# PereUbu7/Variational-Self-Organizing-Maps

Hardware: AMD Instinct MI355X
Metric: training samples/sec per epoch (BMU+update), 128x128 map, 784-dim (higher is better)
Workload: dtype f32

## Files before the change

variational-self-organizing-maps_amd/csrc/vsom_device.hpp:

```cpp
#pragma once
#include "vsom_internal.hpp"

struct DistArgs {
    const float *xa;
    const float *xb;
    int ldx;
    const float *ma;
    const float *mb;
    int ldm;
    int L;
};

template <bool CLR>
__device__ __forceinline__ float vsom_resid(float x, float y, float m, float b)
{
    if (CLR) {
        float t = m * x;
        t = t + b;
        t = t - y;
        return t;
    }
    return m - x;
}

// ... 115 lines not shown
__device__ __forceinline__ void vsom_local_walk_with(DistFn dist, u64 width, u64 height, u64 start, int lane,
                                                     u64 &minIndexOut, float &minDistOut)
{
    const int g = lane >> 3, k = lane & 7;
    const u64 m1 = ~0ull;
    const u64 fsx = (g == 0 || g >= 6) ? m1 : ((g == 1 || g == 5) ? 0ull : 1ull);
    const u64 fsy = (g <= 2) ? 1ull : ((g == 3 || g == 7) ? 0ull : m1);

    u64 lastBMU = start;
    float minDist = dist(lastBMU, k);
    minDist = __shfl(minDist, 0);
    u64 minIndex = lastBMU;
    u64 lastMeasured = lastBMU;

    for (;;) {
        const u64 lmX = lastMeasured % width, lmY = lastMeasured / width;
        const u64 lbX = lastBMU % width, lbY = lastBMU / width;
        if (lastMeasured == lastBMU) {
            u64 cx = lmX + fsx;
            cx = cx < width - 1 ? cx : width - 1;
            u64 cy = lmY + fsy;
            cy = cy < height - 1 ? cy : height - 1;
            u64 node = cy * width + cx;
            float d = dist(node, k);
#pragma unroll
            for (int i = 0; i < 8; ++i) {
                float di = __shfl(d, i * 8);
                u64 ni = __shfl(node, i * 8);
                if (di < minDist) {
                    minDist = di;
                    minIndex = ni;
                }
            }
            if (minIndex == lastBMU)
                break;
            lastMeasured = minIndex;
        } else {
            if (lmX - lbX) {
                u64 cx = lmX + lmX - lbX;
                cx = cx < width - 1 ? cx : width - 1;
                u64 off = (u64)(long long)((g < 3 ? g : 0) - 1);
                u64 cy = lmY + off;
                cy = cy < height - 1 ? cy : height - 1;
                u64 node = cy * width + cx;
                float d = dist(node, k);
#pragma unroll
                for (int i = 0; i < 3; ++i) {
                    float di = __shfl(d, i * 8);
                    u64 ni = __shfl(node, i * 8);
                    if (di < minDist) {
                        minDist = di;
                        minIndex = ni;
                    }
                }
            }
            (void)lbY;
            if (minIndex == lastMeasured)
                break;
            lastBMU = lastMeasured;
            lastMeasured = minIndex;
        }
    }
    minIndexOut = minIndex;
    minDistOut = minDist;
}

template <bool CLR>
__device__ __forceinline__ void vsom_local_walk(const DistArgs &a, const float *xa, const float *xb, u64 width,
                                                u64 height, u64 start, int lane, u64 &minIndexOut, float &minDistOut)
{
    vsom_local_walk_with(
        [&](u64 node, int k) {
            return vsom_group_dist<CLR>(xa, xb, a.ma + (size_t)node * a.ldm, a.mb + (size_t)node * a.ldm, a.L, k);
        },
        width, height, start, lane, minIndexOut, minDistOut);
}

__device__ __forceinline__ void vsom_somindex(u64 idx, u64 W, u64 H, int &x, int &y)
{
    u64 xm = idx % W;
    x = (int)xm;
    y = (int)((idx - xm) / H);
}
```

variational-self-organizing-maps_amd/csrc/vsom_internal.hpp:

```cpp
#pragma once

#include <hip/hip_runtime.h>
#include <stdint.h>
#include <stddef.h>
#include <algorithm>
#include <map>
#include <string>
#include <tuple>
#include <vector>

#include "../../include/vsom_hip.h"
#include "vsom_buf.hpp"

typedef unsigned long long u64;

#define VSOM_CHAIN_MAX_WAVES 448

#define VSOM_TK 32

constexpr size_t VSOM_ROW_PAD = 32;
constexpr size_t VSOM_ONL_STATE_BYTES = 4352;

struct vsom_custom_state;

// ... 34 lines not shown
    DevBuf<int> cc_idx_alt, cc_inv_alt;
    DevBuf<unsigned> cc_meta_alt;
    hipEvent_t ev_rows_free = nullptr, ev_ahead = nullptr;
    bool rows_free_valid = false;
    bool ahead_valid = false;
    bool ahead_rows = false;
    size_t ahead_B = 0;
    bool ahead_cc = false, ahead_xi = false;
    const float *next_dev = nullptr;
    size_t next_dev_B = 0;
    bool next_dev_pending = false;
    PinnedBuf<float> mse;
    PinnedBuf<unsigned char> sch_host; DevBuf<unsigned char> sch_dev;
    PinnedBuf<float> sch_mse;
    DevBuf<int> pair_i, pair_j;

    DevBuf<u64> partial;
    DevBuf<unsigned char> nan0;

    DevBuf<u64> dd_hash; DevBuf<int> dd_rep, dd_list;
    bool dedupe = true;
    double dd_min_work = 2.0e10;
    bool tiny_lds_attr[12] = {};

    DevBuf<float> sl_G, sl_nrm; DevBuf<unsigned> sl_scal;
    DevBuf<float> sl_a2;
    DevBuf<int> sl_list;
    DevBuf<float> sl_tmin;
    PinnedBuf<unsigned> sl_fb;
    DevBuf<float> sl_fs, sl_fm;
    DevBuf<signed char> sl_xi; DevBuf<float> sl_l1;
    DevBuf<signed char> sl_q; DevBuf<double> sl_qscale, sl_qcorr;
    DevBuf<int4> sl_qfast;
    uint32_t sl_kp8 = 0;
    bool xi_valid = false;
    int sl_par = 0;
    int sl_skip = 0;
    unsigned sl_seq_seen = 0;
    int sl_fail_streak = 0;

    DevBuf<float2> cw;
    DevBuf<float> lut; PinnedBuf<float> lut_host;
    hipEvent_t lut_ev[2] = {nullptr, nullptr}; bool lut_ev_valid[2] = {false, false}; int lut_slot = 0;
    double lut_sigma = -1.0; uint32_t lut_w = 0, lut_h = 0;
    DevBuf<double> lutd; double lutd_sigma = -1.0;
    PinnedBuf<double> lutd_host; double lutd_host_sigma[2] = {-1.0, -1.0};
    hipEvent_t lutd_ev[2] = {nullptr, nullptr}; bool lutd_ev_valid[2] = {false, false}; int lutd_slot = 0;

    void *upd_module = nullptr, *upd_clr8 = nullptr;
    void *upd_quad[VSOM_QF_COUNT][VSOM_QV_COUNT] = {};
    bool mean_nt4 = false;
    int update_mode = VSOM_UPDATE_STRICT;
    bool use_chain = true;
    bool use_tiny = true;

    DevBuf<unsigned> cc_flags;
    DevBuf<int> cc_idx;
    DevBuf<int> cc_inv;
    DevBuf<unsigned> cc_meta;
    PinnedBuf<unsigned> cc_fb;
    unsigned cc_seen = 0;
    int cc_skip = 0;
    long cc_min_rows = 1024;
    bool cc_valid = false;
    uint32_t cpitch = 0;
    DevBuf<float> Xc;
    DevBuf<float> Mc;
    DevBuf<float> Uc_map, Uc_S;
    DevBuf<float4> Xq;
    DevBuf<unsigned> zq;
    bool xq_valid = false;
    uint32_t xq_bpad = 0, xq_quads = 0;

    struct PendingSigma {
        bool on = false;
        size_t B = 0;
        uint32_t bpad = 0;
        bool compact = false;
        VsomQuadVariant variant = VSOM_QV_STD;
        double sigma = 0.0;
    } sg;
    DevBuf<int> sg_inv; DevBuf<unsigned> sg_meta;
    DevBuf<u64> sg_bmu;
    int sigma_mode = VSOM_SIGMA_AUTO;
    unsigned sigma_unread = 0;
    bool sigma_shared = false;
    uint64_t sg_stats[3] = {0, 0, 0};

    DevBuf<float> v_dev;
    PinnedBuf<float> v_pinned;
    DevBuf<float> res_dev;
    DevBuf<u64> onl_state;
    DevBuf<float> onl_f;
    DevBuf<unsigned char> onl_img; DevBuf<float4> onl_nsc; DevBuf<float> onl_lb; DevBuf<unsigned> onl_u;
    DevBuf<float4> onl_xsc;
    DevBuf<unsigned char> onl_dirty;

    PinnedBuf<float> st_pinned;
    PinnedBuf<u64> out_pinned;
    DevBuf<unsigned char> q_scratch;
    PinnedBuf<unsigned char> q_pinned;
    DevBuf<double> umatrix;
    bool um_valid = false;

    uint32_t timing = 0;
    struct Ev { hipEvent_t a, b; int which; };
    std::vector<Ev> ev_live;
    std::vector<Ev> ev_pool;
    float t_ms[VSOM_T_COUNT] = {0};
    uint32_t t_cnt[VSOM_T_COUNT] = {0};

    bool in_group = false;

    vsom_custom_state *cu = nullptr;
};

void vsom_set_error(const std::string &msg);
int vsom_fail(int code, const std::string &msg);
#define VSOM_HIP_CHECK_AS(expr, what)                                                    \
    do {                                                                                 \
        hipError_t _e = (expr);                                                          \
        if (_e != hipSuccess) {                                                          \
            (void)hipGetLastError();                                                     \
            return vsom_fail(_e == hipErrorOutOfMemory ? VSOM_ERR_NOMEM : VSOM_ERR_HIP,  \
                             std::string(what) + ": " + hipGetErrorString(_e));          \
        }                                                                                \
    } while (0)
#define VSOM_HIP_CHECK(expr) VSOM_HIP_CHECK_AS(expr, #expr)
#define VSOM_ALLOC_CHECK(expr) VSOM_HIP_CHECK_AS(expr, "hipMalloc in " #expr)

struct TimerScope {
    vsom_ctx *c; int which; vsom_ctx::Ev ev; bool on;
    TimerScope(vsom_ctx *ctx, int w);
    ~TimerScope();
};

struct DistArgs;
DistArgs vsom_dist_args(const vsom_ctx *c);
struct VsomNodeGroups {
    size_t G, ng;
};
inline VsomNodeGroups vsom_node_groups(size_t ntiles, size_t rtiles, size_t maxg)
{
    const size_t want = std::min<size_t>({maxg, ntiles, std::max<size_t>(1, (2048 + rtiles - 1) / rtiles)});
    const size_t G = (ntiles + want - 1) / want;
    return {G, (ntiles + G - 1) / G};
}
int launch_stage_chunk(vsom_ctx *c, const float *x_dev, size_t B);
int ensure_chunk_capacity(vsom_ctx *c, size_t B);
bool vsom_can_stage_ahead(const vsom_ctx *c, size_t B);
int launch_stage_chunk_ahead(vsom_ctx *c, const float *x_dev, size_t B);
int vsom_adopt_ahead(vsom_ctx *c);
int vsom_prefetch_rows(vsom_ctx *c, const float *x_host, size_t B, size_t r0, size_t r1);
int vsom_commit_begin(vsom_ctx *c, float **raw, size_t *B);
int vsom_commit_end(vsom_ctx *c);
int launch_bmu_full(vsom_ctx *c, size_t s0, size_t s1);
int launch_bmu_local(vsom_ctx *c, size_t s0, size_t s1);
int launch_pair_dist(vsom_ctx *c, const u64 *nodes_dev, const u64 *rows_dev, size_t count,
                     float *out_dev);
int launch_finish(vsom_ctx *c);
int vsom_join_aux(vsom_ctx *c);
int vsom_join_aux_keep(vsom_ctx *c);
int vsom_sigma_flush_pending(vsom_ctx *c);
void vsom_sigma_drop(vsom_ctx *c);
int launch_bmu_restricted(vsom_ctx *c, u64 min_hits);
int launch_row_dist(vsom_ctx *c, size_t row, float *out_dev);
// ... 101 lines not shown
```

variational-self-organizing-maps_amd/csrc/vsom_update.hip:

```cpp
#include "vsom_device.hpp"
#include "vsom_phase2_plan.hpp"
#include <algorithm>
#include <cmath>
#include <cstdlib>
#include <mutex>


#define CWP_WT 512
#define CWP_THREADS (64 + CWP_WT)
template <int NW, int T, bool LUT_LDS, bool CONLY>
__global__ __launch_bounds__(CWP_THREADS) void cwp_kernel(const u64 *__restrict__ lastbmu, int B, int n0, int n1,
                                                          int W, int H, const float *__restrict__ lut,
                                                          int lutw, int luth, float2 *__restrict__ cw, int ldn,
                                                          float *__restrict__ weight)
{
    static_assert(NW * T == 2048 && CWP_WT % NW == 0 && T % 4 == 0 && T <= CWP_WT, "worker mapping");
    constexpr int LK = NW * T / CWP_WT;
    constexpr int PK = LK / 2;
    constexpr int QK = LK / 4;
    static_assert(LK % 4 == 0, "whole sample quads per worker thread");
    constexpr int SS = CWP_WT / NW;
    extern __shared__ __attribute__((aligned(16))) unsigned char cwp_smem[];
    float *wL = (float *)cwp_smem;
    float *WL = wL + 3 * T * NW;
    int2 *bL = (int2 *)(WL + 2 * T * NW);
    float *slut = (float *)(bL + 3 * T);
    const int tid = threadIdx.x;
    if (LUT_LDS) {
        for (int i = tid; i < lutw * luth; i += CWP_THREADS)
            slut[i] = lut[i];
    }
    const float *tab = LUT_LDS ? slut : lut;
    const int ntiles = (B + T - 1) / T;
    const int nloc = n1 - n0;
    const int wt = tid - 64;
    const int lnode = (wt < 0 ? tid : wt) & (NW - 1);
    const int s0 = wt < 0 ? 0 : wt / NW;
    const int nl = blockIdx.x * NW + lnode;
    const bool valid = nl < nloc;
    int cx = 0, cy = 0;
    if (valid)
        vsom_somindex((u64)(n0 + nl), (u64)W, (u64)H, cx, cy);

    auto load_bxy = [&](int t) {
        if (t < ntiles && wt < T) {
            const int j = t * T + wt;
            int bx = 0, by = 0;
            if (j < B)
                vsom_somindex(lastbmu[j], (u64)W, (u64)H, bx, by);
            bL[(t % 3) * T + wt] = make_int2(bx, by);
        }
    };
    auto lookup = [&](int t) {
        float *dst = wL + (t % 3) * T * NW;
        const int2 *bsrc = bL + (t % 3) * T;
        const int nt = B - t * T < T ? B - t * T : T;
        int2 b[LK];
        float w[LK];
#pragma unroll
        for (int k = 0; k < LK; ++k)
            b[k] = bsrc[s0 + k * SS];
#pragma unroll
        for (int k = 0; k < LK; ++k) {
            int dx = cx - b[k].x, dy = cy - b[k].y;
            dx = dx < 0 ? -dx : dx;
            dy = dy < 0 ? -dy : dy;
            dx = dx < lutw ? dx : lutw - 1;
            dy = dy < luth ? dy : luth - 1;
            w[k] = tab[dy * lutw + dx];
        }
#pragma unroll
        for (int k = 0; k < LK; ++k)
            if (s0 + k * SS < nt)
                dst[(s0 + k * SS) * NW + lnode] = w[k];
    };
    auto emit = [&](int t) {
        const float *ws = wL + (t % 3) * T * NW;
        const float *Ws = WL + (t & 1) * T * NW;
        const int nt = B - t * T < T ? B - t * T : T;
        if (CONLY) {
            float w[QK][4], Wp[QK][4];
#pragma unroll
            for (int k = 0; k < QK; ++k) {
                const int s = (s0 + k * SS) * 4;
#pragma unroll
                for (int i = 0; i < 4; ++i) {
                    w[k][i] = ws[(s + i) * NW + lnode];
                    Wp[k][i] = Ws[(s + i) * NW + lnode];
                }
            }
#pragma unroll
            for (int k = 0; k < QK; ++k) {
                const int s = (s0 + k * SS) * 4;
                float4 o;
                o.x = w[k][0] / Wp[k][0];
                o.y = s + 1 < nt ? w[k][1] / Wp[k][1] : 0.f;
                o.z = s + 2 < nt ? w[k][2] / Wp[k][2] : 0.f;
                o.w = s + 3 < nt ? w[k][3] / Wp[k][3] : 0.f;
                if (valid && s < nt)
                    ((float4 *)cw)[(size_t)((t * T + s) >> 2) * ldn + nl] = o;
            }
            return;
        }
        float w0[PK], w1[PK], W0[PK], W1[PK];
#pragma unroll
        for (int k = 0; k < PK; ++k) {
            const int s = (s0 + k * SS) * 2;
            w0[k] = ws[s * NW + lnode];
            W0[k] = Ws[s * NW + lnode];
            w1[k] = ws[(s + 1) * NW + lnode];
            W1[k] = Ws[(s + 1) * NW + lnode];
        }
#pragma unroll
        for (int k = 0; k < PK; ++k) {
            const int s = (s0 + k * SS) * 2;
            float4 o;
            o.x = w0[k] / W0[k];
            o.y = w0[k];
            const bool two = s + 1 < nt;
            o.z = two ? w1[k] / W1[k] : 0.f;
            o.w = two ? w1[k] : 0.f;
            if (valid && s < nt)
                ((float4 *)cw)[(size_t)((t * T + s) >> 1) * ldn + nl] = o;
        }
    };

    float run = 0.f;
    if (wt >= 0) {
        load_bxy(0);
        load_bxy(1);
    }
    __syncthreads();
    if (wt >= 0)
        lookup(0);
    __syncthreads();
    for (int t = 0; t < ntiles; ++t) {
        if (wt >= 0) {
            load_bxy(t + 2);
            if (t + 1 < ntiles)
                lookup(t + 1);
            if (t > 0)
                emit(t - 1);
        } else {
            const float *ws = wL + (t % 3) * T * NW;
            float *Ws = WL + (t & 1) * T * NW;
            const int nt = B - t * T < T ? B - t * T : T;
            int s = 0;
            for (; s + 16 <= nt; s += 16) {
                float r[16], o[16];
#pragma unroll
                for (int k = 0; k < 16; ++k)
                    r[k] = ws[(s + k) * NW + lnode];
#pragma unroll
                for (int k = 0; k < 16; ++k) {
                    run = run + r[k];
                    o[k] = run;
                }
                if (tid < NW) {
#pragma unroll
                    for (int k = 0; k < 16; ++k)
                        Ws[(s + k) * NW + lnode] = o[k];
                }
            }
            for (; s < nt; ++s) {
                run = run + ws[s * NW + lnode];
                if (tid < NW)
                    Ws[s * NW + lnode] = run;
            }
        }
        __syncthreads();
    }
    if (wt >= 0)
        emit(ntiles - 1);
    else if (tid < NW && valid && weight)
        weight[n0 + nl] = run;
}

typedef float vsom_f2 __attribute__((ext_vector_type(2)));

#define VSOM_MED_STEP(XS, CW)                                                                    \
    "v_pk_fma_f32 %[t], %[M], %[k24], " XS " neg_lo:[0,1,0] neg_hi:[0,1,0]\n\t"                   \
    "v_pk_mul_f32 %[p], %[t], %[k127] clamp\n\t"                                                  \
    "v_pk_mul_f32 %[n], %[t], %[k127] neg_lo:[1,0] neg_hi:[1,0] clamp\n\t"                        \
    "v_pk_fma_f32 %[M], " CW ", %[p], %[M] op_sel_hi:[0,1,1]\n\t"                                 \
    "v_pk_fma_f32 %[S], " CW ", %[p], %[S] op_sel:[1,0,0]\n\t"                                    \
    "v_pk_fma_f32 %[M], " CW ", %[n], %[M] op_sel_hi:[0,1,1] neg_lo:[1,0,0] neg_hi:[1,0,0]\n\t"   \
    "v_pk_fma_f32 %[S], " CW ", %[n], %[S] op_sel:[1,0,0]\n\t"

__device__ __forceinline__ void vsom_median_steps8(vsom_f2 &M, vsom_f2 &S, const vsom_f2 (&xs)[8], const float4 (&cv)[4])
{
    const vsom_f2 k24 = {0x1.0p24f, 0x1.0p24f}, k127 = {0x1.0p127f, 0x1.0p127f};
    const vsom_f2 c0 = {cv[0].x, cv[0].y}, c1 = {cv[0].z, cv[0].w}, c2 = {cv[1].x, cv[1].y}, c3 = {cv[1].z, cv[1].w},
                  c4 = {cv[2].x, cv[2].y}, c5 = {cv[2].z, cv[2].w}, c6 = {cv[3].x, cv[3].y}, c7 = {cv[3].z, cv[3].w};
    vsom_f2 t, p, n;
    asm volatile(VSOM_MED_STEP("%[x0]", "%[c0]") VSOM_MED_STEP("%[x1]", "%[c1]") VSOM_MED_STEP("%[x2]", "%[c2]")
                 VSOM_MED_STEP("%[x3]", "%[c3]") VSOM_MED_STEP("%[x4]", "%[c4]") VSOM_MED_STEP("%[x5]", "%[c5]")
                 VSOM_MED_STEP("%[x6]", "%[c6]") VSOM_MED_STEP("%[x7]", "%[c7]")
                 : [M] "+v"(M), [S] "+v"(S), [t] "=&v"(t), [p] "=&v"(p), [n] "=&v"(n)
                 : [x0] "v"(xs[0]), [x1] "v"(xs[1]), [x2] "v"(xs[2]), [x3] "v"(xs[3]), [x4] "v"(xs[4]), [x5] "v"(xs[5]),
                   [x6] "v"(xs[6]), [x7] "v"(xs[7]), [c0] "v"(c0), [c1] "v"(c1), [c2] "v"(c2), [c3] "v"(c3), [c4] "v"(c4),
                   [c5] "v"(c5), [c6] "v"(c6), [c7] "v"(c7), [k24] "s"(k24), [k127] "s"(k127));
}

__device__ __forceinline__ void vsom_median_step1(vsom_f2 &M, vsom_f2 &S, vsom_f2 xs, vsom_f2 cw)
{
    const vsom_f2 k24 = {0x1.0p24f, 0x1.0p24f}, k127 = {0x1.0p127f, 0x1.0p127f};
    vsom_f2 t, p, n;
    asm volatile(VSOM_MED_STEP("%[x0]", "%[c0]")
                 : [M] "+v"(M), [S] "+v"(S), [t] "=&v"(t), [p] "=&v"(p), [n] "=&v"(n)
                 : [x0] "v"(xs), [c0] "v"(cw), [k24] "s"(k24), [k127] "s"(k127));
}

template <bool MEDIAN, int FMA, int PLOG>
__global__ __launch_bounds__(256, 1) void update_chain3_kernel(const float *__restrict__ Xs, int ldx,
                                                               const float2 *__restrict__ cw, int ldn, int B,
                                                               int n0, int nloc, int D,
                                                               float *__restrict__ map,
                                                               float *__restrict__ sigma, int pitch,
                                                               const float *__restrict__ weight)
{
    constexpr int PL = 1 << PLOG, NW = 256 >> PLOG, CT = 64;
    constexpr int XP = CT * PL / 2 / 256;
    constexpr int CP = (CT / 2) * NW / 256 > 0 ? (CT / 2) * NW / 256 : 1;
    static_assert(PLOG >= 3 && PLOG <= 6, "8..64 dim pairs per node row");
    __shared__ __attribute__((aligned(16))) float xs[3][CT][2 * PL];
    __shared__ __attribute__((aligned(16))) float4 cs[3][CT / 2][NW];
    if (MEDIAN)
        asm volatile("s_setreg_imm32_b32 hwreg(HW_REG_MODE, 8, 1), 0");
    const int tid = threadIdx.x;
    const int lnode = tid >> PLOG, lp = tid & (PL - 1);
    const int nl = blockIdx.x * NW + lnode;
    const int d = 2 * (blockIdx.y * PL + lp);
    const bool valid = nl < nloc && d < D;
    const int nbase = blockIdx.x * NW;
    const float *xbase = Xs + 2 * blockIdx.y * PL;
    const int nblocks = (B + CT - 1) / CT;
    const int lastrow = B > 0 ? B - 1 : 0, lastpair = B > 0 ? (B - 1) >> 1 : 0;

    auto load_x = [&](int blk, int i) {
        const int piece = tid + 256 * i;
        int row = blk * CT + piece / (PL / 2);
        row = row < lastrow ? row : lastrow;
        return *reinterpret_cast<const float4 *>(xbase + (size_t)row * ldx + 4 * (piece % (PL / 2)));
    };
    auto load_c = [&](int blk, int i) {
        int piece = tid + 256 * i;
        piece = piece < (CT / 2) * NW ? piece : (CT / 2) * NW - 1;
        int pr = blk * (CT / 2) + piece / NW;
        pr = pr < lastpair ? pr : lastpair;
        int node = nbase + piece % NW;
// ... 194 lines not shown
    c->upd_clr8 = f;
    static const char *const quad_names[VSOM_QF_COUNT][VSOM_QV_COUNT] = {
        {"std_nt4", "fma_nt4", "sfma_nt4", "med_nt4"},
        {"mean_nt4", "meanfma_nt4", "mean_nt4", "medmean_nt4"},
        {"mean_nt8", "meanfma_nt8", "mean_nt8", "medmean_nt8"}};
    for (int form = 0; form < VSOM_QF_COUNT; ++form)
        for (int v = 0; v < VSOM_QV_COUNT; ++v) {
            const std::string n = std::string("vsom_update_") + quad_names[form][v] + "_gfx950";
            VSOM_HIP_CHECK(hipModuleGetFunction(&f, mod, n.c_str()));
            c->upd_quad[form][v] = f;
        }
#ifdef VSOM_DEVELOPMENT
    c->mean_nt4 = std::getenv("VSOM_MEAN_NT4") != nullptr;
#endif
    c->upd_module = mod;
    return VSOM_OK;
}

double vsom_neighbourhood_weight(size_t cx, size_t cy, size_t bx, size_t by, double sigma)
{
    if (sigma > 1.0) {
        double cxd = (double)cx, cyd = (double)cy, bxd = (double)bx, byd = (double)by;
        return std::exp(-((cxd - bxd) * (cxd - bxd) / 2.0 / sigma / sigma +
                          (cyd - byd) * (cyd - byd) / 2.0 / sigma / sigma));
    } else if (cx == bx && cy == by) {
        return 1.0;
    }
    return 0.0;
}

int ensure_lut(vsom_ctx *c, double sigma)
{
    if (c->lut.p && c->lut_sigma == sigma)
        return VSOM_OK;
    uint32_t ymax = c->N ? (c->N - c->W) / c->H : 0;
    uint32_t lh = ymax + 1, lw = c->W;
    size_t need = (size_t)lh * lw;
    if (need > c->lut.cap) {
        VSOM_HIP_CHECK(hipStreamSynchronize(c->stream));
        VSOM_ALLOC_CHECK(vsom_grow_set(c->stream, 0, {vsom_member(c->lut, need), vsom_member(c->lut_host, 2 * need)}));
        c->lut_ev_valid[0] = c->lut_ev_valid[1] = false;
    }
    const int k = c->lut_slot;
    c->lut_slot ^= 1;
    if (!c->lut_ev[k])
        VSOM_HIP_CHECK(hipEventCreateWithFlags(&c->lut_ev[k], hipEventDisableTiming));
    if (c->lut_ev_valid[k])
        VSOM_HIP_CHECK(hipEventSynchronize(c->lut_ev[k]));
    float *host = c->lut_host.p + (size_t)k * c->lut.cap;
    for (uint32_t dy = 0; dy < lh; ++dy)
        for (uint32_t dx = 0; dx < lw; ++dx)
            host[(size_t)dy * lw + dx] = (float)vsom_neighbourhood_weight(dx, dy, 0, 0, sigma);
    VSOM_HIP_CHECK(hipMemcpyAsync(c->lut.p, host, need * sizeof(float), hipMemcpyHostToDevice, c->stream));
    VSOM_HIP_CHECK(hipEventRecord(c->lut_ev[k], c->stream));
    c->lut_ev_valid[k] = true;
    c->lut_sigma = sigma;
    c->lut_w = lw;
    c->lut_h = lh;
    return VSOM_OK;
}

__global__ void empty_epoch_kernel(float *__restrict__ map, float *__restrict__ sigma, float *__restrict__ weight,
                                   int pitch, int part_pitch, int part_len, int n0, int nloc)
{
    const size_t i = (size_t)blockIdx.x * blockDim.x + threadIdx.x;
    if (i >= (size_t)nloc * pitch)
        return;
    const int nl = (int)(i / pitch), col = (int)(i % pitch);
    const size_t at = (size_t)(n0 + nl) * pitch + col;
    const float zero = weight[n0 + nl] * 0.f;
    map[at] = 0.f;
    sigma[at] = (col % part_pitch) < part_len ? sqrtf(0.f / (zero * 0.f + 0.f)) : 0.f;
}

__global__ void zero_weight_kernel(float *__restrict__ weight, int n0, int nloc)
{
    const int i = blockIdx.x * blockDim.x + threadIdx.x;
    if (i < nloc)
        weight[n0 + i] = 0.f;
}

extern "C" int vsom_small_map_chains(const vsom_ctx *c, size_t nodes) { return c && vsom_use_chain(*c, nodes) ? 1 : 0; }

static int launch_cwp(vsom_ctx *c, const u64 *bmu, size_t B_, size_t n0, size_t n1, size_t ldn, bool conly, float *weight)
{
    const size_t nloc = n1 - n0;
    const size_t lut_bytes = (size_t)c->lut_w * c->lut_h * sizeof(float);
    const bool lds = lut_bytes <= 24 * 1024;
    constexpr int nw = 16, T = 2048 / nw;
    const size_t smem = (size_t)5 * 2048 * sizeof(float) + (size_t)3 * T * sizeof(int2) + (lds ? lut_bytes : 0);
    const void *fn = conly ? (lds ? (const void *)cwp_kernel<nw, T, true, true> : (const void *)cwp_kernel<nw, T, false, true>)
                           : (lds ? (const void *)cwp_kernel<nw, T, true, false> : (const void *)cwp_kernel<nw, T, false, false>);
    if (smem > 64 * 1024)
        VSOM_HIP_CHECK(hipFuncSetAttribute(fn, hipFuncAttributeMaxDynamicSharedMemorySize, (int)smem));
    int B = (int)B_, in0 = (int)n0, in1 = (int)n1, iW = (int)c->W, iH = (int)c->H, lw = (int)c->lut_w, lh = (int)c->lut_h,
        ildn = (int)ldn;
    const float *lut = c->lut.p;
    float2 *cwp = c->cw.p;
    void *args[] = {&bmu, &B, &in0, &in1, &iW, &iH, &lut, &lw, &lh, &cwp, &ildn, &weight};
    VSOM_HIP_CHECK(hipLaunchKernel(fn, dim3((unsigned)((nloc + nw - 1) / nw)), dim3(CWP_THREADS), args, smem, c->stream));
    return VSOM_OK;
}

static int launch_nt_chains(vsom_ctx *c, const Phase2Plan &p, size_t n0, size_t B, uint32_t bpad, const unsigned *meta)
{
    const unsigned cols = p.compact ? c->cpitch : c->pitch;
    UpdAsmArgs a;
    a.xs = c->Xq.p;
    a.cw2 = c->cw.p;
    a.map = p.compact ? c->Uc_map.p : c->map.p;
    a.sbuf = p.compact ? c->Uc_S.p : c->sigma.p;
    a.ldx_bytes = bpad * 16u;
    a.ldn_bytes = (unsigned)(p.ldn * 16u);
    a.B = (unsigned)B;
    a.nloc = (unsigned)p.nloc;
    a.nslices = p.quads;
    a.pitch_bytes = cols * 4u;
    a.n0 = (unsigned)n0;
    a.ppitch_bytes = 0;
    a.yp = p.compact ? (const void *)meta : nullptr;
    a.zq = c->zq.p;
    size_t sz = 80;
    void *extra[] = {HIP_LAUNCH_PARAM_BUFFER_POINTER, &a, HIP_LAUNCH_PARAM_BUFFER_SIZE, &sz, HIP_LAUNCH_PARAM_END};
    VSOM_HIP_CHECK(hipModuleLaunchKernel((hipFunction_t)c->upd_quad[p.form][p.variant], p.grid_x, p.grid_y, 1, p.block, 1, 1, 0,
                                         c->stream, nullptr, extra));
    return VSOM_OK;
}

static int run_after(vsom_ctx *c, const Phase2Plan &p, size_t n0, const int *inv = nullptr)
{
    if (p.after == VSOM_P2_NOTHING)
        return VSOM_OK;
    TimerScope ts(c, VSOM_T_SIGMA);
    if (p.after != VSOM_P2_FINALIZE_COLUMNS)
        return vsom_cc_expand(c, n0, p.nloc,
                              p.after == VSOM_P2_EXPAND_MAP_ONLY ? VSOM_EXPAND_MAP
                              : p.after == VSOM_P2_EXPAND_SIGMA_ONLY ? VSOM_EXPAND_SIGMA : VSOM_EXPAND_BOTH, inv);
    for (uint32_t part = 0; part < c->nparts; ++part)
        hipLaunchKernelGGL(sigma_finalize_kernel, dim3((unsigned)p.nloc), dim3(256), 0, c->stream, c->sigma.p, c->map.p,
                           (int)c->pitch, (int)(part * c->part_pitch), (int)p.after_cols, (int)c->part_len, (int)n0, (int)p.nloc,
                           c->weight.p);
    VSOM_HIP_CHECK(hipGetLastError());
    return VSOM_OK;
}

__global__ __launch_bounds__(256) void sg_keep_record_kernel(const int *__restrict__ inv, int ninv, const unsigned *__restrict__ meta,
                                                             int *__restrict__ inv_out, unsigned *__restrict__ meta_out,
                                                             const u64 *__restrict__ bmu, int nb, u64 *__restrict__ bmu_out)
{
    const int i = blockIdx.x * blockDim.x + threadIdx.x;
    if (i < ninv)
        inv_out[i] = inv[i];
    if (i < 16 && ninv > 0)
        meta_out[i] = meta[i];
    if (i < nb)
        bmu_out[i] = bmu[i];
}

void vsom_sigma_drop(vsom_ctx *c)
{
    if (c->sg.on) {
        c->sg.on = false;
        ++c->sg_stats[1];
    }
}

static int sigma_materialise(vsom_ctx *c)
{
    const vsom_ctx::PendingSigma p = c->sg;
    int rc = ensure_lut(c, p.sigma);
    if (rc)
        return rc;
    c->sg.on = false;
    ++c->sg_stats[2];
    const Phase2Plan plan = vsom_phase2_replay(*c, p.B, p.variant, p.compact);
    {
        TimerScope ts(c, VSOM_T_CW);
        if ((rc = launch_cwp(c, c->sg_bmu.p, p.B, 0, c->N, plan.ldn, false, nullptr)))
            return rc;
    }
    {
        TimerScope ts(c, VSOM_T_UPDATE);
        if ((rc = launch_nt_chains(c, plan, 0, p.B, p.bpad, c->sg_meta.p)))
            return rc;
    }
    return run_after(c, plan, 0, c->sg_inv.p);
}

int vsom_sigma_flush_pending(vsom_ctx *c)
{
    c->sigma_unread = 0;
    return c->sg.on ? sigma_materialise(c) : VSOM_OK;
}

static int run_clr(vsom_ctx *c, const Phase2Plan &p, size_t n0)
{
    UpdAsmArgs a;
    a.xs = c->XP.p;
    a.cw2 = c->cw.p;
    a.map = c->map.p;
    a.sbuf = c->sigma.p;
    a.ldx_bytes = c->part_pitch * 4u;
    a.ldn_bytes = (unsigned)(p.ldn * 16u);
    a.B = (unsigned)c->B;
    a.nloc = (unsigned)p.nloc;
    a.nslices = p.nslices;
    a.pitch_bytes = c->pitch * 4u;
    a.n0 = (unsigned)n0;
    a.ppitch_bytes = c->part_pitch * 4u;
    a.yp = c->YP.p;
    a.zq = nullptr;
    size_t sz = 72;
    void *extra[] = {HIP_LAUNCH_PARAM_BUFFER_POINTER, &a, HIP_LAUNCH_PARAM_BUFFER_SIZE, &sz, HIP_LAUNCH_PARAM_END};
    VSOM_HIP_CHECK(hipModuleLaunchKernel((hipFunction_t)c->upd_clr8, p.grid_x, p.grid_y, 1, p.block, 1, 1, 0, c->stream, nullptr,
                                         extra));
    return VSOM_OK;
}

static int run_small_map(vsom_ctx *c, const Phase2Plan &p, size_t n0)
{
    using K3 = void (*)(const float *, int, const float2 *, int, int, int, int, int, float *, float *, int, const float *);
    static constexpr K3 k3[VSOM_QV_COUNT][4] = {
        {update_chain3_kernel<false, 0, 3>, update_chain3_kernel<false, 0, 4>, update_chain3_kernel<false, 0, 5>, update_chain3_kernel<false, 0, 6>},
        {update_chain3_kernel<false, 1, 3>, update_chain3_kernel<false, 1, 4>, update_chain3_kernel<false, 1, 5>, update_chain3_kernel<false, 1, 6>},
        {update_chain3_kernel<false, 2, 3>, update_chain3_kernel<false, 2, 4>, update_chain3_kernel<false, 2, 5>, update_chain3_kernel<false, 2, 6>},
        {update_chain3_kernel<true, 0, 3>, update_chain3_kernel<true, 0, 4>, update_chain3_kernel<true, 0, 5>, update_chain3_kernel<true, 0, 6>}};
    const float *xs_ = c->Xs.p;
    const float2 *cw_ = c->cw.p;
    int ildx = (int)c->xpitch, ildn = (int)p.ldn, iB = (int)c->B, in0 = (int)n0, inl = (int)p.nloc, iD = (int)c->D,
        ipitch = (int)c->pitch;
    float *map_ = c->map.p, *sg_ = c->sigma.p;
    const float *wt_ = c->weight.p;
    void *args[] = {&xs_, &ildx, &cw_, &ildn, &iB, &in0, &inl, &iD, &map_, &sg_, &ipitch, &wt_};
    VSOM_HIP_CHECK(hipLaunchKernel((const void *)k3[p.variant][p.pl_log2 - 3], dim3(p.grid_x, p.grid_y), dim3(p.block), args, 0,
                                   c->stream));
    return VSOM_OK;
}

static int run_quads(vsom_ctx *c, const Phase2Plan &p, double sigma, size_t n0)
{
    int rc = vsom_xq_ensure(c);
    if (rc)
        return rc;
    if (p.offer_rows_free) {
        VSOM_HIP_CHECK(hipEventRecord(c->ev_rows_free, c->stream));
        c->rows_free_valid = true;
    }
    if (p.compact && (rc = vsom_cc_ensure_update_scratch(c)))
        return rc;
    if (!p.deferred)
        return launch_nt_chains(c, p, n0, c->B, c->xq_bpad, c->cc_meta.p);
    hipLaunchKernelGGL(sg_keep_record_kernel, dim3((unsigned)((std::max<size_t>(p.compact ? c->xpitch : 0, c->B) + 255) / 256)),
                       dim3(256), 0, c->stream, c->cc_inv.p, p.compact ? (int)c->xpitch : 0, c->cc_meta.p, c->sg_inv.p,
                       c->sg_meta.p, c->lastbmu.p, (int)c->B, c->sg_bmu.p);
    if ((rc = launch_nt_chains(c, p, n0, c->B, c->xq_bpad, c->cc_meta.p)))
        return rc;
    c->sg.on = true;
    c->sg.B = c->B;
    c->sg.bpad = c->xq_bpad;
    c->sg.compact = p.compact;
    c->sg.variant = p.variant;
    c->sg.sigma = sigma;
    ++c->sg_stats[0];
    return VSOM_OK;
}

int launch_phase2(vsom_ctx *c, double sigma, size_t n0, size_t n1, bool may_defer)
{
    if (n1 <= n0)
        return vsom_join_aux_keep(c);
    const bool full = n0 == 0 && n1 == c->N;
    if (c->sg.on && !full)
        if (int prc = sigma_materialise(c))
            return prc;
    auto done = [&]() {
        if (may_defer && full && c->sigma_unread < 1000u)
            ++c->sigma_unread;
        return vsom_join_aux_keep(c);
    };
    if (c->B == 0) {
        TimerScope ts(c, VSOM_T_UPDATE);
        const size_t nloc = n1 - n0, tot = nloc * c->pitch;
        hipLaunchKernelGGL(empty_epoch_kernel, dim3((unsigned)((tot + 255) / 256)), dim3(256), 0, c->stream, c->map.p,
                           c->sigma.p, c->weight.p, (int)c->pitch, (int)c->part_pitch, (int)c->part_len, (int)n0, (int)nloc);
        hipLaunchKernelGGL(zero_weight_kernel, dim3((unsigned)((nloc + 255) / 256)), dim3(256), 0, c->stream, c->weight.p,
                           (int)n0, (int)nloc);
        VSOM_HIP_CHECK(hipGetLastError());
        vsom_sigma_drop(c);
        return done();
    }
    int rc = ensure_lut(c, sigma);
    if (rc)
        return rc;
    if ((rc = vsom_load_asm_module(c)))
        return rc;
    const Phase2Plan plan = vsom_phase2_plan(*c, n0, n1, may_defer);
    vsom_sigma_drop(c);
    if (plan.deferred) {
        if (plan.compact)
            VSOM_ALLOC_CHECK(vsom_grow_set(c->stream, 0, {vsom_member(c->sg_inv, c->xpitch), vsom_member(c->sg_meta, 16)}));
        VSOM_ALLOC_CHECK(vsom_grow(c->sg_bmu, c->B, c->stream));
    }
    VSOM_ALLOC_CHECK(vsom_grow(c->cw, plan.cw_elems, c->stream, VSOM_BUF_ZERO));
    {
        TimerScope ts(c, VSOM_T_CW);
        if ((rc = launch_cwp(c, c->lastbmu.p, c->B, n0, n1, plan.ldn, plan.deferred, c->weight.p)))
            return rc;
    }
    {
        TimerScope ts(c, VSOM_T_UPDATE);
        if (plan.reads_staged_rows)
            c->rows_free_valid = false;
        rc = plan.path == VSOM_P2_CLR ? run_clr(c, plan, n0)
             : plan.path == VSOM_P2_SMALL_MAP ? run_small_map(c, plan, n0) : run_quads(c, plan, sigma, n0);
        if (rc)
            return rc;
        VSOM_HIP_CHECK(hipGetLastError());
    }
    if ((rc = run_after(c, plan, n0)))
        return rc;
    return done();
}
```

Before: 1.806 million.

## Precompute BMU coordinates in a pre-pass and retune the neighbourhood-weight kernel

Adds a small kernel that turns each BMU index into (x,y) coordinates once, replacing the per-workgroup 64-bit modulo/divide inside the weight kernel. The old sg_keep_record copy work is folded into that same kernel, so the launch count stays the same. The weight kernel becomes templated on worker count and uses fewer worker threads (384) when there are many workgroups. It also uses 32-bit index math and umul24 LUT addressing, and gains full-tile specialisations that drop bounds checks and run a double-buffered prefix scan. In exchange there is an extra int2 buffer, a dependency on the pre-pass, a new LUT size guard, and more kernel instantiations.

```diff
diff --git a/variational-self-organizing-maps_amd/csrc/vsom_device.hpp b/variational-self-organizing-maps_amd/csrc/vsom_device.hpp
--- a/variational-self-organizing-maps_amd/csrc/vsom_device.hpp
+++ b/variational-self-organizing-maps_amd/csrc/vsom_device.hpp
@@ -221,3 +221,10 @@
     x = (int)xm;
     y = (int)((idx - xm) / H);
 }
+
+__device__ __forceinline__ void vsom_somindex32(unsigned idx, unsigned W, unsigned H, int &x, int &y)
+{
+    unsigned xm = idx % W;
+    x = (int)xm;
+    y = (int)((idx - xm) / H);
+}
diff --git a/variational-self-organizing-maps_amd/csrc/vsom_internal.hpp b/variational-self-organizing-maps_amd/csrc/vsom_internal.hpp
--- a/variational-self-organizing-maps_amd/csrc/vsom_internal.hpp
+++ b/variational-self-organizing-maps_amd/csrc/vsom_internal.hpp
@@ -140,6 +140,7 @@
     } sg;
     DevBuf<int> sg_inv; DevBuf<unsigned> sg_meta;
     DevBuf<u64> sg_bmu;
+    DevBuf<int2> bxy;
     int sigma_mode = VSOM_SIGMA_AUTO;
     unsigned sigma_unread = 0;
     bool sigma_shared = false;
diff --git a/variational-self-organizing-maps_amd/csrc/vsom_update.hip b/variational-self-organizing-maps_amd/csrc/vsom_update.hip
--- a/variational-self-organizing-maps_amd/csrc/vsom_update.hip
+++ b/variational-self-organizing-maps_amd/csrc/vsom_update.hip
@@ -4,22 +4,23 @@
 #include <cmath>
 #include <cstdlib>
 #include <mutex>
+#include <type_traits>
 
 
 #define CWP_WT 512
-#define CWP_THREADS (64 + CWP_WT)
-template <int NW, int T, bool LUT_LDS, bool CONLY>
-__global__ __launch_bounds__(CWP_THREADS) void cwp_kernel(const u64 *__restrict__ lastbmu, int B, int n0, int n1,
+#define CWP_WT_MANY 384
+template <int NW, int T, bool LUT_LDS, bool CONLY, int WT>
+__global__ __launch_bounds__(64 + WT) void cwp_kernel(const int2 *__restrict__ bxy, int B, int n0, int n1,
                                                           int W, int H, const float *__restrict__ lut,
                                                           int lutw, int luth, float2 *__restrict__ cw, int ldn,
                                                           float *__restrict__ weight)
 {
-    static_assert(NW * T == 2048 && CWP_WT % NW == 0 && T % 4 == 0 && T <= CWP_WT, "worker mapping");
-    constexpr int LK = NW * T / CWP_WT;
+    static_assert(NW * T == 4 * WT && WT % NW == 0 && T % 8 == 0 && T <= WT, "worker mapping");
+    constexpr int LK = NW * T / WT;
     constexpr int PK = LK / 2;
     constexpr int QK = LK / 4;
     static_assert(LK % 4 == 0, "whole sample quads per worker thread");
-    constexpr int SS = CWP_WT / NW;
+    constexpr int SS = WT / NW;
     extern __shared__ __attribute__((aligned(16))) unsigned char cwp_smem[];
     float *wL = (float *)cwp_smem;
     float *WL = wL + 3 * T * NW;
@@ -27,7 +28,7 @@
     float *slut = (float *)(bL + 3 * T);
     const int tid = threadIdx.x;
     if (LUT_LDS) {
-        for (int i = tid; i < lutw * luth; i += CWP_THREADS)
+        for (int i = tid; i < lutw * luth; i += 64 + WT)
             slut[i] = lut[i];
     }
     const float *tab = LUT_LDS ? slut : lut;
@@ -40,21 +41,17 @@
     const bool valid = nl < nloc;
     int cx = 0, cy = 0;
     if (valid)
-        vsom_somindex((u64)(n0 + nl), (u64)W, (u64)H, cx, cy);
+        vsom_somindex32((unsigned)(n0 + nl), (unsigned)W, (unsigned)H, cx, cy);
 
     auto load_bxy = [&](int t) {
         if (t < ntiles && wt < T) {
             const int j = t * T + wt;
-            int bx = 0, by = 0;
-            if (j < B)
-                vsom_somindex(lastbmu[j], (u64)W, (u64)H, bx, by);
-            bL[(t % 3) * T + wt] = make_int2(bx, by);
+            bL[(t % 3) * T + wt] = j < B ? bxy[j] : make_int2(0, 0);
         }
     };
     auto lookup = [&](int t) {
         float *dst = wL + (t % 3) * T * NW;
         const int2 *bsrc = bL + (t % 3) * T;
-        const int nt = B - t * T < T ? B - t * T : T;
         int2 b[LK];
         float w[LK];
 #pragma unroll
@@ -67,18 +64,20 @@
             dy = dy < 0 ? -dy : dy;
             dx = dx < lutw ? dx : lutw - 1;
             dy = dy < luth ? dy : luth - 1;
-            w[k] = tab[dy * lutw + dx];
+            w[k] = *(const float *)((const char *)tab + ((__umul24(dy, lutw) + (unsigned)dx) << 2));
         }
 #pragma unroll
         for (int k = 0; k < LK; ++k)
-            if (s0 + k * SS < nt)
-                dst[(s0 + k * SS) * NW + lnode] = w[k];
-    };
-    auto emit = [&](int t) {
+            dst[(s0 + k * SS) * NW + lnode] = w[k];
+    };
+    float4 *const out0 = (float4 *)cw + ((size_t)s0 * ldn + nl);
+    auto emit_tile = [&](int t, auto full_tile) {
+        constexpr bool FULL = decltype(full_tile)::value;
         const float *ws = wL + (t % 3) * T * NW;
         const float *Ws = WL + (t & 1) * T * NW;
-        const int nt = B - t * T < T ? B - t * T : T;
+        const int nt = FULL ? T : B - t * T;
         if (CONLY) {
+            float4 *const out = out0 + (size_t)(t * (T / 4)) * ldn;
             float w[QK][4], Wp[QK][4];
 #pragma unroll
             for (int k = 0; k < QK; ++k) {
@@ -94,14 +93,15 @@
                 const int s = (s0 + k * SS) * 4;
                 float4 o;
                 o.x = w[k][0] / Wp[k][0];
-                o.y = s + 1 < nt ? w[k][1] / Wp[k][1] : 0.f;
-                o.z = s + 2 < nt ? w[k][2] / Wp[k][2] : 0.f;
-                o.w = s + 3 < nt ? w[k][3] / Wp[k][3] : 0.f;
-                if (valid && s < nt)
-                    ((float4 *)cw)[(size_t)((t * T + s) >> 2) * ldn + nl] = o;
+                o.y = FULL || s + 1 < nt ? w[k][1] / Wp[k][1] : 0.f;
+                o.z = FULL || s + 2 < nt ? w[k][2] / Wp[k][2] : 0.f;
+                o.w = FULL || s + 3 < nt ? w[k][3] / Wp[k][3] : 0.f;
+                if (valid && (FULL || s < nt))
+                    out[(size_t)(k * SS) * ldn] = o;
             }
             return;
         }
+        float4 *const out = out0 + (size_t)(t * (T / 2)) * ldn;
         float w0[PK], w1[PK], W0[PK], W1[PK];
 #pragma unroll
         for (int k = 0; k < PK; ++k) {
@@ -117,15 +117,23 @@
             float4 o;
             o.x = w0[k] / W0[k];
             o.y = w0[k];
-            const bool two = s + 1 < nt;
+            const bool two = FULL || s + 1 < nt;
             o.z = two ? w1[k] / W1[k] : 0.f;
             o.w = two ? w1[k] : 0.f;
-            if (valid && s < nt)
-                ((float4 *)cw)[(size_t)((t * T + s) >> 1) * ldn + nl] = o;
-        }
+            if (valid && (FULL || s < nt))
+                out[(size_t)(k * SS) * ldn] = o;
+        }
+    };
+    auto emit = [&](int t) {
+        if (B - t * T >= T)
+            emit_tile(t, std::true_type());
+        else
+            emit_tile(t, std::false_type());
     };
 
     float run = 0.f;
+    if (wt < 0)
+        __builtin_amdgcn_s_setprio(3);
     if (wt >= 0) {
         load_bxy(0);
         load_bxy(1);
@@ -141,10 +149,34 @@
                 lookup(t + 1);
             if (t > 0)
                 emit(t - 1);
-        } else {
+        } else if (tid < NW) {
             const float *ws = wL + (t % 3) * T * NW;
             float *Ws = WL + (t & 1) * T * NW;
             const int nt = B - t * T < T ? B - t * T : T;
+            if (nt == T) {
+                constexpr int CB = 8;
+                float r[2][CB];
+#pragma unroll
+                for (int k = 0; k < CB; ++k)
+                    r[0][k] = ws[k * NW + lnode];
+#pragma unroll
+                for (int b = 0; b < T / CB; ++b) {
+                    if (b + 1 < T / CB) {
+#pragma unroll
+                        for (int k = 0; k < CB; ++k)
+                            r[(b + 1) & 1][k] = ws[((b + 1) * CB + k) * NW + lnode];
+                    }
+                    float o[CB];
+#pragma unroll
+                    for (int k = 0; k < CB; ++k) {
+                        run = run + r[b & 1][k];
+                        o[k] = run;
+                    }
+#pragma unroll
+                    for (int k = 0; k < CB; ++k)
+                        Ws[(b * CB + k) * NW + lnode] = o[k];
+                }
+            } else {
             int s = 0;
             for (; s + 16 <= nt; s += 16) {
                 float r[16], o[16];
@@ -156,16 +188,14 @@
                     run = run + r[k];
                     o[k] = run;
                 }
-                if (tid < NW) {
-#pragma unroll
-                    for (int k = 0; k < 16; ++k)
-                        Ws[(s + k) * NW + lnode] = o[k];
-                }
+#pragma unroll
+                for (int k = 0; k < 16; ++k)
+                    Ws[(s + k) * NW + lnode] = o[k];
             }
             for (; s < nt; ++s) {
                 run = run + ws[s * NW + lnode];
-                if (tid < NW)
-                    Ws[s * NW + lnode] = run;
+                Ws[s * NW + lnode] = run;
+            }
             }
         }
         __syncthreads();
@@ -526,23 +556,67 @@
 
 extern "C" int vsom_small_map_chains(const vsom_ctx *c, size_t nodes) { return c && vsom_use_chain(*c, nodes) ? 1 : 0; }
 
-static int launch_cwp(vsom_ctx *c, const u64 *bmu, size_t B_, size_t n0, size_t n1, size_t ldn, bool conly, float *weight)
+__global__ __launch_bounds__(256) void bmu_coords_kernel(const u64 *__restrict__ bmu, int nb, int W, int H, int2 *__restrict__ xy,
+                                                         u64 *__restrict__ bmu_out, const int *__restrict__ inv, int ninv,
+                                                         const unsigned *__restrict__ meta, int *__restrict__ inv_out,
+                                                         unsigned *__restrict__ meta_out)
+{
+    const int i = blockIdx.x * blockDim.x + threadIdx.x;
+    if (i < ninv)
+        inv_out[i] = inv[i];
+    if (i < 16 && ninv > 0)
+        meta_out[i] = meta[i];
+    if (i < nb) {
+        const u64 idx = bmu[i];
+        int x, y;
+        if (idx >> 32)
+            vsom_somindex(idx, (u64)W, (u64)H, x, y);
+        else
+            vsom_somindex32((unsigned)idx, (unsigned)W, (unsigned)H, x, y);
+        xy[i] = make_int2(x, y);
+        if (bmu_out)
+            bmu_out[i] = idx;
+    }
+}
+
+static int launch_bmu_coords(vsom_ctx *c, const u64 *bmu, size_t B, bool keep, bool compact)
+{
+    VSOM_ALLOC_CHECK(vsom_grow(c->bxy, B, c->stream));
+    const int ninv = keep && compact ? (int)c->xpitch : 0;
+    hipLaunchKernelGGL(bmu_coords_kernel, dim3((unsigned)((std::max<size_t>((size_t)ninv, B) + 255) / 256)), dim3(256), 0, c->stream,
+                       bmu, (int)B, (int)c->W, (int)c->H, c->bxy.p, keep ? c->sg_bmu.p : nullptr, c->cc_inv.p, ninv, c->cc_meta.p,
+                       c->sg_inv.p, c->sg_meta.p);
+    VSOM_HIP_CHECK(hipGetLastError());
+    return VSOM_OK;
+}
+
+static int launch_cwp(vsom_ctx *c, size_t B_, size_t n0, size_t n1, size_t ldn, bool conly, float *weight)
 {
     const size_t nloc = n1 - n0;
     const size_t lut_bytes = (size_t)c->lut_w * c->lut_h * sizeof(float);
+    if (lut_bytes >= ((size_t)1 << 32) || c->lut_w >= (1u << 24) || c->lut_h >= (1u << 24))
+        return vsom_fail(VSOM_ERR_INVALID, "the neighbourhood table of this map exceeds 4 GiB");
     const bool lds = lut_bytes <= 24 * 1024;
-    constexpr int nw = 16, T = 2048 / nw;
-    const size_t smem = (size_t)5 * 2048 * sizeof(float) + (size_t)3 * T * sizeof(int2) + (lds ? lut_bytes : 0);
-    const void *fn = conly ? (lds ? (const void *)cwp_kernel<nw, T, true, true> : (const void *)cwp_kernel<nw, T, false, true>)
-                           : (lds ? (const void *)cwp_kernel<nw, T, true, false> : (const void *)cwp_kernel<nw, T, false, false>);
+    constexpr int nw = 16;
+    const size_t wgs = (nloc + nw - 1) / nw;
+    const bool many = wgs > 768;
+    const int wt = many ? CWP_WT_MANY : CWP_WT, T = 4 * wt / nw;
+    const size_t smem = (size_t)5 * nw * T * sizeof(float) + (size_t)3 * T * sizeof(int2) + (lds ? lut_bytes : 0);
+    static const void *const fns[2][2][2] = {
+        {{(const void *)cwp_kernel<nw, 4 * CWP_WT / nw, false, false, CWP_WT>, (const void *)cwp_kernel<nw, 4 * CWP_WT / nw, true, false, CWP_WT>},
+         {(const void *)cwp_kernel<nw, 4 * CWP_WT / nw, false, true, CWP_WT>, (const void *)cwp_kernel<nw, 4 * CWP_WT / nw, true, true, CWP_WT>}},
+        {{(const void *)cwp_kernel<nw, 4 * CWP_WT_MANY / nw, false, false, CWP_WT_MANY>, (const void *)cwp_kernel<nw, 4 * CWP_WT_MANY / nw, true, false, CWP_WT_MANY>},
+         {(const void *)cwp_kernel<nw, 4 * CWP_WT_MANY / nw, false, true, CWP_WT_MANY>, (const void *)cwp_kernel<nw, 4 * CWP_WT_MANY / nw, true, true, CWP_WT_MANY>}}};
+    const void *fn = fns[many][conly][lds];
     if (smem > 64 * 1024)
         VSOM_HIP_CHECK(hipFuncSetAttribute(fn, hipFuncAttributeMaxDynamicSharedMemorySize, (int)smem));
     int B = (int)B_, in0 = (int)n0, in1 = (int)n1, iW = (int)c->W, iH = (int)c->H, lw = (int)c->lut_w, lh = (int)c->lut_h,
         ildn = (int)ldn;
     const float *lut = c->lut.p;
     float2 *cwp = c->cw.p;
-    void *args[] = {&bmu, &B, &in0, &in1, &iW, &iH, &lut, &lw, &lh, &cwp, &ildn, &weight};
-    VSOM_HIP_CHECK(hipLaunchKernel(fn, dim3((unsigned)((nloc + nw - 1) / nw)), dim3(CWP_THREADS), args, smem, c->stream));
+    const int2 *bxy = c->bxy.p;
+    void *args[] = {&bxy, &B, &in0, &in1, &iW, &iH, &lut, &lw, &lh, &cwp, &ildn, &weight};
+    VSOM_HIP_CHECK(hipLaunchKernel(fn, dim3((unsigned)wgs), dim3(64 + wt), args, smem, c->stream));
     return VSOM_OK;
 }
 
@@ -588,19 +662,6 @@
     return VSOM_OK;
 }
 
-__global__ __launch_bounds__(256) void sg_keep_record_kernel(const int *__restrict__ inv, int ninv, const unsigned *__restrict__ meta,
-                                                             int *__restrict__ inv_out, unsigned *__restrict__ meta_out,
-                                                             const u64 *__restrict__ bmu, int nb, u64 *__restrict__ bmu_out)
-{
-    const int i = blockIdx.x * blockDim.x + threadIdx.x;
-    if (i < ninv)
-        inv_out[i] = inv[i];
-    if (i < 16 && ninv > 0)
-        meta_out[i] = meta[i];
-    if (i < nb)
-        bmu_out[i] = bmu[i];
-}
-
 void vsom_sigma_drop(vsom_ctx *c)
 {
     if (c->sg.on) {
@@ -620,7 +681,7 @@
     const Phase2Plan plan = vsom_phase2_replay(*c, p.B, p.variant, p.compact);
     {
         TimerScope ts(c, VSOM_T_CW);
-        if ((rc = launch_cwp(c, c->sg_bmu.p, p.B, 0, c->N, plan.ldn, false, nullptr)))
+        if ((rc = launch_bmu_coords(c, c->sg_bmu.p, p.B, false, false)) || (rc = launch_cwp(c, p.B, 0, c->N, plan.ldn, false, nullptr)))
             return rc;
     }
     {
@@ -694,9 +755,6 @@
         return rc;
     if (!p.deferred)
         return launch_nt_chains(c, p, n0, c->B, c->xq_bpad, c->cc_meta.p);
-    hipLaunchKernelGGL(sg_keep_record_kernel, dim3((unsigned)((std::max<size_t>(p.compact ? c->xpitch : 0, c->B) + 255) / 256)),
-                       dim3(256), 0, c->stream, c->cc_inv.p, p.compact ? (int)c->xpitch : 0, c->cc_meta.p, c->sg_inv.p,
-                       c->sg_meta.p, c->lastbmu.p, (int)c->B, c->sg_bmu.p);
     if ((rc = launch_nt_chains(c, p, n0, c->B, c->xq_bpad, c->cc_meta.p)))
         return rc;
     c->sg.on = true;
@@ -748,7 +806,8 @@
     VSOM_ALLOC_CHECK(vsom_grow(c->cw, plan.cw_elems, c->stream, VSOM_BUF_ZERO));
     {
         TimerScope ts(c, VSOM_T_CW);
-        if ((rc = launch_cwp(c, c->lastbmu.p, c->B, n0, n1, plan.ldn, plan.deferred, c->weight.p)))
+        if ((rc = launch_bmu_coords(c, c->lastbmu.p, c->B, plan.deferred, plan.compact)) ||
+            (rc = launch_cwp(c, c->B, n0, n1, plan.ldn, plan.deferred, c->weight.p)))
             return rc;
     }
     {
```

Result: no change. 1.822 million, median of 4 (+0.9%).
